# Kudo510/ImageSequenceRegistrationfor6DPoseEstimationLabeling

Hardware: AMD Instinct MI355X
Metric: registered images/sec (T-LESS obj 1-like, synthetic) + final Chamfer error (higher is better)
Workload: dtype bf16

## Files before the change

imagesequenceregistrationfor6dposeestimationlabeling_amd/_capi.py:

```python
from __future__ import annotations

import ctypes as C
from pathlib import Path

import torch

import os

_PKG = Path(__file__).resolve().parent
LIB_PATH = Path(os.environ["ISR_HIP_LIB"]) if os.environ.get("ISR_HIP_LIB") else _PKG / "libisr_hip.so"

ISR_OK = 0
ABI_VERSION = 6
DTYPE_BF16 = 0
DTYPE_F32 = 1
DTYPE_BF16_LOG2 = 2
DTYPE_BF16_LOG2_SCREENED = 3
RANSAC_STAGED = 0
RANSAC_SEQUENTIAL = 1
INLIERS_REFIT = 0
INLIERS_RANSAC = 1
FINAL_REFIT = 0
FINAL_EPNP = 1
TUNE = {"nn_path": 0, "nn_filter": 1, "icp_warm": 2, "nn_plan_rq": 3, "nn_plan_blocks": 4,
# ... 131 lines not shown

RADIUS_SIGNATURES = {
    "isr_radius_workspace_bytes": (_sz, [_i]),
    "isr_radius_count": (_i, [_vp, _i, _d, _i, _vp, _vp, _sz, _vp]),
    "isr_radius_count_host": (_i, [_vp, _i, _d, _i, _vp]),
}

KNN_SIGNATURES = {
    "isr_knn_workspace_bytes": (_sz, [_i, _i, _i]),
    "isr_knn": (_i, [_vp, _i, _vp, _i, _i, _vp, _vp, _vp, _sz, _vp]),
    "isr_knn_host": (_i, [_vp, _i, _vp, _i, _i, _vp, _vp]),
    "isr_local_frames": (_i, [_vp, _i, _vp, _i, _i, _vp, _vp, _vp]),
    "isr_local_frames_host": (_i, [_vp, _i, _vp, _i, _i, _vp, _vp]),
}

_RAYS_SPEC = [_i, _vp, _vp, _vp, _vp, _i, _i, _i, _i, _i, _f, _f, _f, _f, _f, _f, _i, _u64]
RAYS_SIGNATURES = {
    "isr_rays_workspace_bytes": (_sz, [_i, _i]),
    "isr_rays_bundle": (_i, [*_RAYS_SPEC, _vp, _vp, _vp, _vp, _vp]),
    "isr_rays_bundle_host": (_i, [*_RAYS_SPEC, _vp, _vp, _vp, _vp]),
    "isr_rays_select_count": (_i, [*_RAYS_SPEC, _vp, _i, _i, _vp, _vp, _sz, _vp]),
    "isr_rays_select_emit": (_i, [*_RAYS_SPEC, _vp, _i, _i, _vp, _sz, _i64, _vp, _vp, _vp, _vp, _vp, _vp]),
    "isr_rays_select_count_host": (_i, [*_RAYS_SPEC, _vp, _i, _i, _vp]),
    "isr_rays_select_emit_host": (_i, [*_RAYS_SPEC, _vp, _i, _i, _i64, _vp, _vp, _vp, _vp, _vp]),
    "isr_sample_nearest": (_i, [_vp, _i, _i, _i, _i, _vp, _i, _vp, _vp]),
    "isr_sample_nearest_host": (_i, [_vp, _i, _i, _i, _i, _vp, _i, _vp]),
    "isr_rays_philox_host": (_i, [_vp, _vp, _vp, _vp]),
}

_RADIANCE_FIELD = [_vp, _sz, _i, _vp, _i, _i, _i]
# ... 66 lines not shown
    if _lib is not None:
        return _lib
    if not LIB_PATH.exists():
        raise IsrError(
            f"{LIB_PATH} is missing: build it with "
            "`python -m imagesequenceregistrationfor6dposeestimationlabeling_amd.build` "
            "(there is no CPU fallback)")
    try:
        L = C.CDLL(str(LIB_PATH))
    except OSError as e:
        raise IsrError(f"cannot load {LIB_PATH}: {e}") from e
    for name, (res, args) in {**SIGNATURES, **FIELD_SIGNATURES, **FPS_SIGNATURES, **DENSITY_SIGNATURES,
                               **DENSITY_DIR_SIGNATURES, **RADIUS_SIGNATURES, **MC_SIGNATURES, **KNN_SIGNATURES,
                               **RAYS_SIGNATURES, **RADIANCE_SIGNATURES, **RESAMPLE_SIGNATURES,
                               **CONTRASTIVE_SIGNATURES, **FIELD_GRAD_SIGNATURES, **SAMPLE_GRAD_SIGNATURES,
                               **EA_GRAD_SIGNATURES}.items():
        try:
            fn = getattr(L, name)
        except AttributeError as e:
            raise IsrError(f"{LIB_PATH} does not export {name}") from e
        fn.restype = res
        fn.argtypes = args
    if L.isr_abi_version() != ABI_VERSION:
        raise IsrError(f"ABI version {L.isr_abi_version()} != {ABI_VERSION}")
    _lib = L
    return L


def check(rc: int, what: str) -> None:
    if rc != ISR_OK:
        msg = lib().isr_last_error()
# ... 30 lines not shown
```

imagesequenceregistrationfor6dposeestimationlabeling_amd/csrc/nn_batched.hip:

```cpp
#include "isr_common.hpp"

#include <cstddef>
#include <cstdlib>

namespace {

#ifndef ISR_NN_PACKED_BATCH
#define ISR_NN_PACKED_BATCH 1
#endif
constexpr int kThreads = 256;
constexpr int kTile = 256;
constexpr int kGroup = 8;
constexpr int kNV = 18;

__device__ __forceinline__ void xform64(const double* __restrict__ T, float x, float y, float z,
                                        double& ox, double& oy, double& oz) {
  if (T == nullptr) {
    ox = x; oy = y; oz = z;
    return;
  }
  const double dx = x, dy = y, dz = z;
  ox = fma(T[2], dz, fma(T[1], dy, fma(T[0], dx, T[3])));
  oy = fma(T[6], dz, fma(T[5], dy, fma(T[4], dx, T[7])));
  oz = fma(T[10], dz, fma(T[9], dy, fma(T[8], dx, T[11])));
// ... 886 lines not shown
    else
      nn_finalize_kernel<false><<<fgrid, kThreads, 0, stream>>>(qry, Nq, tgt, Tq, Tt, p.nsplit,
                                                                radius, part_d2, part_idx, b0,
                                                                nn_idx, nn_d, part_sums, nullptr, packed);
    ISR_CHECK_LAUNCH("nn_finalize_kernel");
  }
  if (sum_d || sum_d2 || n_in || cov) {
    const dim3 rblock(32, 8);
    nn_reduce_kernel<<<(B + 7) / 8, rblock, 0, stream>>>(part_sums, p.fblocks, B, sum_d, sum_d2,
                                                         n_in, cov);
    ISR_CHECK_LAUNCH("nn_reduce_kernel");
  }
  return ISR_OK;
}

extern "C" int isr_add_metric(const float* verts, int V, const double* Ta, const double* Tb, int B,
                              double* mean_out, isr_stream_t stream) {
  ISR_REQUIRE(verts && mean_out, "isr_add_metric: null pointer");
  ISR_REQUIRE(V > 0 && B > 0, "isr_add_metric: V=%d B=%d", V, B);
  add_metric_kernel<<<B, kThreads, 0, isr::as_stream(stream)>>>(verts, V, Ta, Tb, mean_out);
  ISR_CHECK_LAUNCH("add_metric_kernel");
  return ISR_OK;
}

extern "C" size_t isr_icp_workspace_bytes(int Ns, int Nt) {
  if (Ns <= 0 || Nt <= 0) return 0;
  const NNPlan p = make_plan(Ns, Nt, 1, true);
  return isr::align_up((size_t)p.fblocks * kNV * sizeof(double), 256) + isr::align_up((size_t)Ns * 8, 256) +
         2 * isr::align_up((size_t)Ns * 4, 256) + isr::align_up((size_t)((Nt + kTile - 1) / kTile) * 6 * sizeof(float), 256) + 2048;
}
// ... 93 lines not shown
```

imagesequenceregistrationfor6dposeestimationlabeling_amd/csrc/nn_grid.hpp:

```cpp
#pragma once

constexpr int kMaxCells = 1 << 20;
constexpr int kMaxRing = 8;

struct GridDesc {
  double gmin[3];
  double h, inv_h;
  int nx, ny, nz, ncell;
};

__global__ __launch_bounds__(1024) void grid_bbox_kernel(const float* __restrict__ tgt, int Nt, double cell_scale,
                                                         GridDesc* __restrict__ g, int32_t* __restrict__ unresolved) {
  __shared__ float smin[3][16], smax[3][16];
  float lo[3] = {3.0e38f, 3.0e38f, 3.0e38f}, hi[3] = {-3.0e38f, -3.0e38f, -3.0e38f};
  for (int j = threadIdx.x; j < Nt; j += blockDim.x) {
#pragma unroll
    for (int a = 0; a < 3; ++a) {
      const float v = tgt[3 * (size_t)j + a];
      lo[a] = fminf(lo[a], v);
      hi[a] = fmaxf(hi[a], v);
    }
  }
#pragma unroll
  for (int a = 0; a < 3; ++a) {
#pragma unroll
    for (int o = 32; o >= 1; o >>= 1) {
      lo[a] = fminf(lo[a], __shfl_xor(lo[a], o, 64));
      hi[a] = fmaxf(hi[a], __shfl_xor(hi[a], o, 64));
// ... 18 lines not shown
    if ((double)nx * ny * nz <= (double)kMaxCells) break;
    h *= 1.26;
  }
  g->h = h; g->inv_h = 1.0 / h;
  g->nx = nx; g->ny = ny; g->nz = nz; g->ncell = nx * ny * nz;
  if (unresolved) *unresolved = 0;
}

__device__ __forceinline__ int grid_axis_cell(double v, double gmin, double inv_h, int n) {
  const double c = floor((v - gmin) * inv_h);
  return c < 0.0 ? 0 : (c > (double)(n - 1) ? n - 1 : (int)c);
}

__global__ __launch_bounds__(kThreads) void grid_count_kernel(const float* __restrict__ tgt, int Nt,
                                                              const GridDesc* __restrict__ g,
                                                              int32_t* __restrict__ cid, int32_t* __restrict__ count) {
  const int j = blockIdx.x * kThreads + threadIdx.x;
  if (j >= Nt) return;
  const int cx = grid_axis_cell(tgt[3 * (size_t)j], g->gmin[0], g->inv_h, g->nx);
  const int cy = grid_axis_cell(tgt[3 * (size_t)j + 1], g->gmin[1], g->inv_h, g->ny);
  const int cz = grid_axis_cell(tgt[3 * (size_t)j + 2], g->gmin[2], g->inv_h, g->nz);
  const int c = (cz * g->ny + cy) * g->nx + cx;
  cid[j] = c;
  atomicAdd(&count[c], 1);
}

__global__ __launch_bounds__(1024) void grid_scan_kernel(const GridDesc* __restrict__ g, const int32_t* __restrict__ count,
                                                         int32_t* __restrict__ start) {
  __shared__ int32_t part[1024];
  const int n = g->ncell;
  const int per = (n + 1023) / 1024;
  const int lo = threadIdx.x * per, hi = min(n, lo + per);
  int32_t s = 0;
  for (int i = lo; i < hi; ++i) s += count[i];
  part[threadIdx.x] = s;
  __syncthreads();
  for (int o = 1; o < 1024; o <<= 1) {
    const int32_t v = threadIdx.x >= o ? part[threadIdx.x - o] : 0;
    __syncthreads();
    part[threadIdx.x] += v;
    __syncthreads();
  }
  int32_t run = threadIdx.x ? part[threadIdx.x - 1] : 0;
  for (int i = lo; i < hi; ++i) { start[i] = run; run += count[i]; }
  if (threadIdx.x == 1023) start[n] = part[1023];
}

__global__ __launch_bounds__(kThreads) void grid_scatter_kernel(const float* __restrict__ tgt, int Nt,
                                                                const int32_t* __restrict__ cid,
                                                                const int32_t* __restrict__ start,
                                                                int32_t* __restrict__ count, float4* __restrict__ sorted) {
  const int j = blockIdx.x * kThreads + threadIdx.x;
  if (j >= Nt) return;
  const int c = cid[j];
  const int pos = start[c] + atomicSub(&count[c], 1) - 1;
  sorted[pos] = make_float4(tgt[3 * (size_t)j], tgt[3 * (size_t)j + 1], tgt[3 * (size_t)j + 2], __int_as_float(j));
}

__global__ __launch_bounds__(kThreads) void nn_grid_search_kernel(
    const float* __restrict__ qry, int Nq, const GridDesc* __restrict__ g, const int32_t* __restrict__ start,
    const float4* __restrict__ sorted, const double* __restrict__ Tq, const double* __restrict__ Tt,
    float stop_radius, float* __restrict__ part_d2, int32_t* __restrict__ part_idx,
    int32_t* __restrict__ unresolved, const int32_t* __restrict__ skip) {
  if (skip && *skip) return;
  const int b = blockIdx.y;
  const int qi = blockIdx.x * kThreads + threadIdx.x;
// ... 83 lines not shown
  } else {
    part_idx[o] = kUnresolved;
    atomicAdd(unresolved, 1);
  }
}

constexpr int kTileRings = 10;
constexpr int kTileRuns = 1024;

struct QBlock {
  int32_t start, count;
};

__global__ __launch_bounds__(kThreads) void qblocks_count_kernel(const GridDesc* __restrict__ g,
                                                                 const int32_t* __restrict__ start, int tb,
                                                                 int32_t* __restrict__ nblk) {
  const int c = blockIdx.x * kThreads + threadIdx.x;
  if (c >= g->ncell) return;
  nblk[c] = (start[c + 1] - start[c] + tb - 1) / tb;
}

__global__ __launch_bounds__(kThreads) void qblocks_fill_kernel(const GridDesc* __restrict__ g,
                                                                const int32_t* __restrict__ start,
                                                                const int32_t* __restrict__ bstart, int tb,
                                                                QBlock* __restrict__ table) {
  const int c = blockIdx.x * kThreads + threadIdx.x;
  if (c >= g->ncell) return;
  const int s0 = start[c], cnt = start[c + 1] - s0;
  int o = bstart[c];
  for (int j = 0; j < cnt; j += tb) table[o++] = QBlock{s0 + j, min(tb, cnt - j)};
}

template <int TB>
__device__ __forceinline__ float block_reduce_max(float v, float* red) {
#pragma unroll
  for (int o = 32; o >= 1; o >>= 1) v = fmaxf(v, __shfl_xor(v, o, 64));
  if (TB == 64) return v;
  __syncthreads();
  if ((threadIdx.x & 63) == 0) red[threadIdx.x >> 6] = v;
  __syncthreads();
  float m = red[0];
#pragma unroll
  for (int w = 1; w < TB / 64; ++w) m = fmaxf(m, red[w]);
  return m;
}

template <int TB>
__global__ __launch_bounds__(TB) void nn_tile_search_kernel(
    const float4* __restrict__ qsorted, const QBlock* __restrict__ qtable, const GridDesc* __restrict__ gq,
    const int32_t* __restrict__ qbstart, int Nq, const GridDesc* __restrict__ g, const int32_t* __restrict__ start,
    const float4* __restrict__ sorted, int Nt, const double* __restrict__ Tq, const double* __restrict__ Tt, int nb,
    float stop_radius, float* __restrict__ part_d2, int32_t* __restrict__ part_idx, const int32_t* __restrict__ skip) {
  __shared__ __attribute__((aligned(16))) float tile[3][kTile];
  __shared__ int32_t tidx[kTile];
  __shared__ int32_t run_start[kTileRuns], run_pref[kTileRuns + 1];
  __shared__ float red[TB / 64];
  __shared__ int32_t scan_w[TB / 64];
  if (skip && *skip) return;
  const int tid = threadIdx.x;
  const int nqb = qbstart[gq->ncell];
  const int nx = g->nx, ny = g->ny, nz = g->nz;
  const double gh = g->h, ginv = g->inv_h;
  const float h = (float)gh;

  for (long item = blockIdx.x; item < (long)nqb * nb; item += gridDim.x) {
    const int b = (int)(item / nqb);
    const QBlock qb = qtable[item % nqb];
    const double* tq = Tq ? Tq + 12 * (size_t)b : nullptr;
    const double* tt = Tt ? Tt + 12 * (size_t)b : nullptr;
    const bool valid = tid < qb.count;
    const float4 qp = qsorted[qb.start + (valid ? tid : 0)];
    const int qorig = __float_as_int(qp.w);
    double x, y, z;
    xform64(tq, qp.x, qp.y, qp.z, x, y, z);
    const float qx = (float)x, qy = (float)y, qz = (float)z;

    double mx = qx, my = qy, mz = qz;
    bool rigid = true;
    if (tt) {
      const double r00 = tt[0], r01 = tt[1], r02 = tt[2], r10 = tt[4], r11 = tt[5], r12 = tt[6], r20 = tt[8],
                   r21 = tt[9], r22 = tt[10];
      const double g00 = r00 * r00 + r10 * r10 + r20 * r20, g11 = r01 * r01 + r11 * r11 + r21 * r21,
                   g22 = r02 * r02 + r12 * r12 + r22 * r22, g01 = r00 * r01 + r10 * r11 + r20 * r21,
                   g02 = r00 * r02 + r10 * r12 + r20 * r22, g12 = r01 * r02 + r11 * r12 + r21 * r22;
      const double dev = fmax(fmax(fmax(fabs(g00 - 1.0), fabs(g11 - 1.0)), fabs(g22 - 1.0)),
                              fmax(fmax(fabs(g01), fabs(g02)), fabs(g12)));
      rigid = dev < 3.0e-3;
// ... 209 lines not shown
         isr::align_up((size_t)(Nq + 1) * sizeof(QBlock), 256);
}

GridWs take_grid(isr::Workspace& w, int Nt) {
  GridWs g;
  char* head = w.take<char>(isr::align_up(sizeof(GridDesc) + 64, 256));
  g.desc = reinterpret_cast<GridDesc*>(head);
  g.unresolved = reinterpret_cast<int32_t*>(head + isr::align_up(sizeof(GridDesc), 16));
  g.count = w.take<int32_t>(kMaxCells + 1);
  g.start = w.take<int32_t>(kMaxCells + 1);
  g.cid = w.take<int32_t>(Nt);
  g.sorted = w.take<float4>(Nt);
  return g;
}

void build_grid(const GridWs& g, const float* tgt, int Nt, hipStream_t stream, double cell_scale = 2.5) {
  (void)hipMemsetAsync(g.count, 0, (size_t)(kMaxCells + 1) * 4, stream);
  grid_bbox_kernel<<<1, 1024, 0, stream>>>(tgt, Nt, cell_scale, g.desc, g.unresolved);
  const int nb = (Nt + kThreads - 1) / kThreads;
  grid_count_kernel<<<nb, kThreads, 0, stream>>>(tgt, Nt, g.desc, g.cid, g.count);
  grid_scan_kernel<<<1, 1024, 0, stream>>>(g.desc, g.count, g.start);
  grid_scatter_kernel<<<nb, kThreads, 0, stream>>>(tgt, Nt, g.cid, g.start, g.count, g.sorted);
}

TileWs take_tile(isr::Workspace& w, int Nq, int Nt) {
  TileWs tw;
  tw.t = take_grid(w, Nt);
  tw.q = take_grid(w, Nq);
  tw.bstart = w.take<int32_t>(kMaxCells + 1);
  tw.table = w.take<QBlock>(Nq + 1);
  return tw;
}

struct TileCfg {
  double st, sq;
  int tb;
};

TileCfg tile_cfg() {
  TileCfg c{kCellScaleTgt, kCellScaleQry, kTileTB};
  if (const int v = isr::tuning(ISR_TUNE_NN_TILE_ST); v > 0) c.st = v * 1e-3;
  if (const int v = isr::tuning(ISR_TUNE_NN_TILE_SQ); v > 0) c.sq = v * 1e-3;
  if (const int v = isr::tuning(ISR_TUNE_NN_TILE_TB); v > 0) c.tb = v;
  if (c.tb != 64 && c.tb != 128 && c.tb != 256) c.tb = kTileTB;
  return c;
}

void build_tile(const TileWs& tw, const float* qry, int Nq, const float* tgt, int Nt, hipStream_t stream) {
  const TileCfg cfg = tile_cfg();
  const double st = cfg.st, sq = cfg.sq;
  const int tb = cfg.tb;
  build_grid(tw.t, tgt, Nt, stream, st);
  build_grid(tw.q, qry, Nq, stream, sq);
  const int cb = (kMaxCells + kThreads - 1) / kThreads;
  (void)hipMemsetAsync(tw.q.count, 0, (size_t)(kMaxCells + 1) * 4, stream);
  qblocks_count_kernel<<<cb, kThreads, 0, stream>>>(tw.q.desc, tw.q.start, tb, tw.q.count);
  grid_scan_kernel<<<1, 1024, 0, stream>>>(tw.q.desc, tw.q.count, tw.bstart);
  qblocks_fill_kernel<<<cb, kThreads, 0, stream>>>(tw.q.desc, tw.q.start, tw.bstart, tb, tw.table);
}

void launch_tile_search(const TileWs& tw, int Nq, int Nt, const double* tq, const double* tt, int nb, float stop_radius,
                        float* part_d2, int32_t* part_idx, const int32_t* skip, hipStream_t stream) {
  const int tb = tile_cfg().tb;
#define ISR_TILE_LAUNCH(TBv)                                                                                      \
  nn_tile_search_kernel<TBv><<<kTileGrid * (kThreads / TBv), TBv, 0, stream>>>(                                   \
      tw.q.sorted, tw.table, tw.q.desc, tw.bstart, Nq, tw.t.desc, tw.t.start, tw.t.sorted, Nt, tq, tt, nb,        \
      stop_radius, part_d2, part_idx, skip)
  if (tb == 64) ISR_TILE_LAUNCH(64);
  else if (tb == 128) ISR_TILE_LAUNCH(128);
  else ISR_TILE_LAUNCH(256);
#undef ISR_TILE_LAUNCH
}
```

imagesequenceregistrationfor6dposeestimationlabeling_amd/ops.py:

```python
from __future__ import annotations

import ctypes
from dataclasses import dataclass

import numpy as np

import torch

from . import _capi
from ._capi import check, current_stream, lib, ptr, require_cuda

_workspaces: dict[tuple, torch.Tensor] = {}

_timers: dict[str, list] | None = None


def enable_timing(on: bool = True) -> None:
    global _timers
    _timers = {} if on else None


def drain_timing() -> dict[str, tuple[int, float, float]]:
    out = {}
    if _timers is None:
# ... 15 lines not shown
            self.e0 = torch.cuda.Event(enable_timing=True)
            self.e1 = torch.cuda.Event(enable_timing=True)
            self.e0.record()
        return self

    def __exit__(self, *exc):
        if _timers is not None:
            self.e1.record()
            _timers.setdefault(self.name, []).append((self.e0, self.e1, self.work))
        return False


class tuning:

    def __init__(self, **knobs):
        self.knobs = {_capi.TUNE[k]: int(v) for k, v in knobs.items()}

    def __enter__(self):
        L = lib()
        self.old = {k: L.isr_tuning_get(k) for k in self.knobs}
        for k, v in self.knobs.items():
            check(L.isr_tuning_set(k, v), "isr_tuning_set")
        return self

    def __exit__(self, *exc):
        L = lib()
        for k, v in self.old.items():
            L.isr_tuning_set(k, v)
        return False


def set_tuning(**knobs) -> None:
    for k, v in knobs.items():
        check(lib().isr_tuning_set(_capi.TUNE[k], int(v)), "isr_tuning_set")


def set_tile_plan(plan: str | None) -> None:
    if plan is None:
        set_tuning(nn_tile_st=0, nn_tile_sq=0, nn_tile_tb=0)
    else:
        st, sq, tb = plan.split(",")
        set_tuning(nn_tile_st=round(float(st) * 1000), nn_tile_sq=round(float(sq) * 1000), nn_tile_tb=int(tb))


def workspace(device: torch.device, nbytes: int, tag: str = "default") -> torch.Tensor:
    key = (device.index, torch.cuda.current_stream(device).cuda_stream, tag)
    buf = _workspaces.get(key)
    if buf is not None and buf.numel() >= nbytes:
        return buf
# ... 45 lines not shown
    L = lib()
    sum_d = torch.empty(B, dtype=torch.float64, device=dev)
    sum_d2 = torch.empty(B, dtype=torch.float64, device=dev)
    n_in = torch.empty(B, dtype=torch.int32, device=dev)
    nn_idx = torch.empty((B, Nq), dtype=torch.int32, device=dev) if want_idx else None
    nn_d = torch.empty((B, Nq), dtype=torch.float64, device=dev) if want_dist else None
    cov = torch.empty((B, 16), dtype=torch.float64, device=dev) if want_cov else None
    nbytes = L.isr_nn_batched_workspace_bytes(Nq, Nt, B)
    ws = workspace(dev, nbytes, "nn")
    with torch.cuda.device(dev), _timed("nn_batched", float(B) * Nq * Nt):
        rc = L.isr_nn_batched(ptr(qry), Nq, ptr(tgt), Nt, ptr(Tq), ptr(Tt), B, float(radius),
                              ptr(sum_d), ptr(sum_d2), ptr(n_in), ptr(nn_idx), ptr(nn_d), ptr(cov),
                              ptr(ws), ws.numel(), current_stream(dev))
    check(rc, "isr_nn_batched")
    return NNResult(sum_d, sum_d2, n_in, nn_idx, nn_d, cov)


def icp_point_to_point_batch(sources: torch.Tensor, target: torch.Tensor, state: torch.Tensor, threshold: float,
                             max_iter: int = 30, rel_fitness: float = 1e-6, rel_rmse: float = 1e-6) -> torch.Tensor:
    dev = require_cuda(sources, target, state)
    if sources.dtype != torch.float32 or target.dtype != torch.float32 or not (sources.is_contiguous() and target.is_contiguous()):
        raise ValueError("icp_point_to_point_batch: sources and target must be contiguous float32")
    if state.dtype != torch.float64 or state.ndim != 2 or state.shape[1] != 20 or not state.is_contiguous():
        raise ValueError(f"icp_point_to_point_batch: state must be contiguous (B,20) float64, got {tuple(state.shape)} {state.dtype}")
    if target.ndim != 2 or target.shape[1] != 3 or sources.ndim not in (2, 3) or sources.shape[-1] != 3:
        raise ValueError(f"icp_point_to_point_batch: sources {tuple(sources.shape)} must be (Ns,3) or (B,Ns,3), target "
                         f"{tuple(target.shape)} (Nt,3)")
    B, Ns, Nt = state.shape[0], sources.shape[-2], target.shape[0]
    if sources.ndim == 3 and sources.shape[0] != B:
        raise ValueError(f"icp_point_to_point_batch: sources {tuple(sources.shape)} and state {tuple(state.shape)} disagree on B")
# ... 1804 lines not shown
```

imagesequenceregistrationfor6dposeestimationlabeling_amd/registration.py:

```python
from __future__ import annotations

import numpy as np
import torch

from . import ops
from ._capi import IsrError

SOLVEPNP_P3P = 2
SOLVEPNP_AP3P = 5

_state = {"surface_pts": None, "device": None}


def device() -> torch.device:
    if not torch.cuda.is_available():
        raise IsrError("no HIP device visible: the registration hot path has no CPU fallback")
    return torch.device("cuda", torch.cuda.current_device())


def _dev(x, dtype=None) -> torch.Tensor:
    if isinstance(x, torch.Tensor):
        t = x if x.is_cuda else x.to(device())
    else:
        t = torch.from_numpy(np.ascontiguousarray(x)).to(device())
# ... 138 lines not shown
    ab = ops.nn_batched(a, b, ta, tb)
    ba = ops.nn_batched(b, a, tb, ta)
    return 0.5 * (float(ab.sum_d.item()) / a.shape[0] + float(ba.sum_d.item()) / b.shape[0])


def chamfer_pairs(pc1, R_pred, R_rel_gt):
    pc = _dev(pc1, torch.float32)
    Rp = np.asarray(R_pred, np.float64)
    Rr = np.asarray(R_rel_gt, np.float64)
    n1 = Rp.shape[0] - 1
    Tg = np.zeros((n1, 3, 4))
    Tp = np.zeros((n1, 3, 4))
    Tg[:, :, :3] = np.einsum("nji,njk->nik", Rr, Rp[:-1])
    Tp[:, :, :3] = np.transpose(Rp[1:], (0, 2, 1))
    tg, tp = _dev(Tg.reshape(n1, 12)), _dev(Tp.reshape(n1, 12))
    ab = ops.nn_batched(pc, pc, tp, tg)
    ba = ops.nn_batched(pc, pc, tg, tp)
    return 0.5 * (ab.sum_d + ba.sum_d) / pc.shape[0]


def choose_best(chamferdis):
    c = chamferdis.cpu().numpy() if isinstance(chamferdis, torch.Tensor) else np.asarray(chamferdis)
    i = int(np.argmin(c))
    return i, float(c[i])


def _eval(src, tgt, threshold, T):
    dev = src.device
    Tq = torch.from_numpy(np.ascontiguousarray(np.asarray(T, np.float64)[:3, :].reshape(1, 12))).to(dev)
    buf = torch.empty(18, dtype=torch.float64, device=dev)
    Nq, Nt = src.shape[0], tgt.shape[0]
    L = ops.lib()
    ws = ops.workspace(dev, L.isr_nn_batched_workspace_bytes(Nq, Nt, 1), "nn")
# ... 167 lines not shown
```

Baseline: 1095.

## Add neighbour-table self-NN path for chamfer between pose-transformed copies of one cloud

Adds a self-nearest-neighbour routine for chamfer between two rigidly transformed copies of the same cloud. It uses a cached per-cloud KNN table and squared radius to resolve most queries cheaply, and runs the exact grid/tile search only for unresolved queries through a device-side 'need' flag. The grid build and tile search kernels gain early-exit guards that read this flag. A Python gate routes to the new path only when most relative rotations are small. This adds KNN table construction, a cache keyed per cloud, and extra kernel launches, and correctness depends on the fallback resolving all misses.

```diff
diff --git a/imagesequenceregistrationfor6dposeestimationlabeling_amd/_capi.py b/imagesequenceregistrationfor6dposeestimationlabeling_amd/_capi.py
--- a/imagesequenceregistrationfor6dposeestimationlabeling_amd/_capi.py
+++ b/imagesequenceregistrationfor6dposeestimationlabeling_amd/_capi.py
@@ -169,6 +169,13 @@
     "isr_local_frames_host": (_i, [_vp, _i, _vp, _i, _i, _vp, _vp]),
 }
 
+NN_SELF_SIGNATURES = {
+    "isr_nn_self_batched_workspace_bytes": (_sz, [_i, _i, _i]),
+    "isr_nn_self_batched": (_i, [_vp, _i, _vp, _vp, _i, _vp, _vp, _i, _d, _vp, _vp, _vp, _vp, _vp, _vp, _vp, _sz, _vp]),
+    "isr_nn_self_search_host": (_i, [_vp, _i, _vp, _vp, _i, _vp, _vp, _i, _vp, _vp, _vp]),
+    "isr_nn_self_unresolved": (_i, [_vp, _sz, _i, _vp, _vp, _vp]),
+}
+
 _RAYS_SPEC = [_i, _vp, _vp, _vp, _vp, _i, _i, _i, _i, _i, _f, _f, _f, _f, _f, _f, _i, _u64]
 RAYS_SIGNATURES = {
     "isr_rays_workspace_bytes": (_sz, [_i, _i]),
@@ -265,7 +272,7 @@
                                **DENSITY_DIR_SIGNATURES, **RADIUS_SIGNATURES, **MC_SIGNATURES, **KNN_SIGNATURES,
                                **RAYS_SIGNATURES, **RADIANCE_SIGNATURES, **RESAMPLE_SIGNATURES,
                                **CONTRASTIVE_SIGNATURES, **FIELD_GRAD_SIGNATURES, **SAMPLE_GRAD_SIGNATURES,
-                               **EA_GRAD_SIGNATURES}.items():
+                               **EA_GRAD_SIGNATURES, **NN_SELF_SIGNATURES}.items():
         try:
             fn = getattr(L, name)
         except AttributeError as e:
diff --git a/imagesequenceregistrationfor6dposeestimationlabeling_amd/csrc/nn_batched.hip b/imagesequenceregistrationfor6dposeestimationlabeling_amd/csrc/nn_batched.hip
--- a/imagesequenceregistrationfor6dposeestimationlabeling_amd/csrc/nn_batched.hip
+++ b/imagesequenceregistrationfor6dposeestimationlabeling_amd/csrc/nn_batched.hip
@@ -1,4 +1,6 @@
 #include "isr_common.hpp"
+#include "nn_self.hpp"
+#include "../../include/isr_nn_self.h"
 
 #include <cstddef>
 #include <cstdlib>
@@ -924,6 +926,83 @@
   return ISR_OK;
 }
 
+namespace {
+NNPlan make_self_plan(int N, int B) {
+  NNPlan p = make_plan(N, N, B);
+  if (p.grid) p.grid = false;
+  p.nsplit = 1;
+  p.split_len = ((N + kTile - 1) / kTile) * kTile;
+  long bc = (long)(kPartBudget / ((size_t)N * 8));
+  p.bchunk = (int)(bc < 1 ? 1 : (bc > B ? B : (bc > 65535 ? 65535 : bc)));
+  return p;
+}
+}
+
+extern "C" size_t isr_nn_self_batched_workspace_bytes(int N, int K, int B) {
+  if (N <= 0 || B <= 0 || K < 1 || K > isr::nn_self::kMaxK || K > N) return 0;
+  const NNPlan p = make_self_plan(N, B);
+  size_t n = isr::nn_self::head_bytes(B);
+  n += isr::align_up((size_t)p.bchunk * N * sizeof(float), 256);
+  n += isr::align_up((size_t)p.bchunk * N * sizeof(int32_t), 256);
+  n += isr::align_up((size_t)B * p.fblocks * kNV * sizeof(double), 256);
+  n += tile_ws_bytes(N, N);
+  return n + 256;
+}
+
+extern "C" int isr_nn_self_batched(const float* pts, int N, const int32_t* nbr, const float* r2, int K, const double* Tq,
+                                   const double* Tt, int B, double radius, double* sum_d, double* sum_d2, int32_t* n_in,
+                                   int32_t* nn_idx, double* nn_d, double* cov, void* ws, size_t ws_bytes, isr_stream_t stream_) {
+  ISR_REQUIRE(pts && nbr && r2, "isr_nn_self_batched: null cloud or table pointer");
+  ISR_REQUIRE(N > 0 && B > 0, "isr_nn_self_batched: N=%d B=%d must be positive", N, B);
+  ISR_REQUIRE(K >= 1 && K <= isr::nn_self::kMaxK && K <= N, "isr_nn_self_batched: K=%d (1..min(N = %d, %d))", K, N,
+              isr::nn_self::kMaxK);
+  ISR_REQUIRE(sum_d || sum_d2 || n_in || nn_idx || nn_d || cov, "isr_nn_self_batched: no output requested");
+  if (!ws || ws_bytes < isr_nn_self_batched_workspace_bytes(N, K, B)) {
+    isr::set_error("isr_nn_self_batched: workspace %zu < %zu", ws_bytes, isr_nn_self_batched_workspace_bytes(N, K, B));
+    return ISR_ERR_WORKSPACE;
+  }
+  hipStream_t stream = isr::as_stream(stream_);
+  const NNPlan p = make_self_plan(N, B);
+  isr::Workspace w(ws, ws_bytes);
+  const isr::nn_self::Head head = isr::nn_self::take_head(w, B);
+  float* part_d2 = w.take<float>((size_t)p.bchunk * N);
+  int32_t* part_idx = w.take<int32_t>((size_t)p.bchunk * N);
+  double* part_sums = w.take<double>((size_t)B * p.fblocks * kNV);
+  TileWs tw{};
+  if (p.tile) tw = take_tile(w, N, N);
+  const float stop_radius = (radius >= 0.0 && !nn_d) ? (float)(radius * (1.0 + 1e-6)) : -1.f;
+
+  for (int b0 = 0; b0 < B; b0 += p.bchunk) {
+    const int nb = (B - b0 < p.bchunk) ? (B - b0) : p.bchunk;
+    const double* tq = Tq ? Tq + 12 * (size_t)b0 : nullptr;
+    const double* tt = Tt ? Tt + 12 * (size_t)b0 : nullptr;
+    if (int rc = isr::nn_self::enqueue(pts, N, nbr, r2, K, Tq, Tt, B, b0, nb, head, part_d2, part_idx, stream)) return rc;
+    if (p.tile) {
+      build_tile(tw, pts, N, pts, N, stream, head.counts);
+      ISR_CHECK_LAUNCH("tile grid build");
+      launch_tile_search(tw, N, N, tq, tt, nb, stop_radius, part_d2, part_idx, nullptr, stream, head.counts, b0);
+    } else {
+      launch_search(p, dim3(p.qblocks, 1, nb), stream, pts, N, pts, N, tq, tt, part_d2, part_idx, nullptr, head.counts, nullptr,
+                    nullptr);
+    }
+    ISR_CHECK_LAUNCH("nn_self exact search");
+    const dim3 fgrid(p.fblocks, nb);
+    if (cov)
+      nn_finalize_kernel<true><<<fgrid, kThreads, 0, stream>>>(pts, N, pts, Tq, Tt, 1, radius, part_d2, part_idx, b0, nn_idx, nn_d,
+                                                               part_sums, nullptr, nullptr);
+    else
+      nn_finalize_kernel<false><<<fgrid, kThreads, 0, stream>>>(pts, N, pts, Tq, Tt, 1, radius, part_d2, part_idx, b0, nn_idx, nn_d,
+                                                                part_sums, nullptr, nullptr);
+    ISR_CHECK_LAUNCH("nn_finalize_kernel");
+  }
+  if (sum_d || sum_d2 || n_in || cov) {
+    const dim3 rblock(32, 8);
+    nn_reduce_kernel<<<(B + 7) / 8, rblock, 0, stream>>>(part_sums, p.fblocks, B, sum_d, sum_d2, n_in, cov);
+    ISR_CHECK_LAUNCH("nn_reduce_kernel");
+  }
+  return ISR_OK;
+}
+
 extern "C" int isr_add_metric(const float* verts, int V, const double* Ta, const double* Tb, int B,
                               double* mean_out, isr_stream_t stream) {
   ISR_REQUIRE(verts && mean_out, "isr_add_metric: null pointer");
diff --git a/imagesequenceregistrationfor6dposeestimationlabeling_amd/csrc/nn_grid.hpp b/imagesequenceregistrationfor6dposeestimationlabeling_amd/csrc/nn_grid.hpp
--- a/imagesequenceregistrationfor6dposeestimationlabeling_amd/csrc/nn_grid.hpp
+++ b/imagesequenceregistrationfor6dposeestimationlabeling_amd/csrc/nn_grid.hpp
@@ -10,8 +10,10 @@
 };
 
 __global__ __launch_bounds__(1024) void grid_bbox_kernel(const float* __restrict__ tgt, int Nt, double cell_scale,
-                                                         GridDesc* __restrict__ g, int32_t* __restrict__ unresolved) {
+                                                         GridDesc* __restrict__ g, int32_t* __restrict__ unresolved,
+                                                         const int32_t* __restrict__ need = nullptr) {
   __shared__ float smin[3][16], smax[3][16];
+  if (need && *need == 0) return;
   float lo[3] = {3.0e38f, 3.0e38f, 3.0e38f}, hi[3] = {-3.0e38f, -3.0e38f, -3.0e38f};
   for (int j = threadIdx.x; j < Nt; j += blockDim.x) {
 #pragma unroll
@@ -60,7 +62,9 @@
 
 __global__ __launch_bounds__(kThreads) void grid_count_kernel(const float* __restrict__ tgt, int Nt,
                                                               const GridDesc* __restrict__ g,
-                                                              int32_t* __restrict__ cid, int32_t* __restrict__ count) {
+                                                              int32_t* __restrict__ cid, int32_t* __restrict__ count,
+                                                              const int32_t* __restrict__ need = nullptr) {
+  if (need && *need == 0) return;
   const int j = blockIdx.x * kThreads + threadIdx.x;
   if (j >= Nt) return;
   const int cx = grid_axis_cell(tgt[3 * (size_t)j], g->gmin[0], g->inv_h, g->nx);
@@ -72,8 +76,10 @@
 }
 
 __global__ __launch_bounds__(1024) void grid_scan_kernel(const GridDesc* __restrict__ g, const int32_t* __restrict__ count,
-                                                         int32_t* __restrict__ start) {
+                                                         int32_t* __restrict__ start,
+                                                         const int32_t* __restrict__ need = nullptr) {
   __shared__ int32_t part[1024];
+  if (need && *need == 0) return;
   const int n = g->ncell;
   const int per = (n + 1023) / 1024;
   const int lo = threadIdx.x * per, hi = min(n, lo + per);
@@ -95,7 +101,9 @@
 __global__ __launch_bounds__(kThreads) void grid_scatter_kernel(const float* __restrict__ tgt, int Nt,
                                                                 const int32_t* __restrict__ cid,
                                                                 const int32_t* __restrict__ start,
-                                                                int32_t* __restrict__ count, float4* __restrict__ sorted) {
+                                                                int32_t* __restrict__ count, float4* __restrict__ sorted,
+                                                                const int32_t* __restrict__ need = nullptr) {
+  if (need && *need == 0) return;
   const int j = blockIdx.x * kThreads + threadIdx.x;
   if (j >= Nt) return;
   const int c = cid[j];
@@ -209,7 +217,9 @@
 
 __global__ __launch_bounds__(kThreads) void qblocks_count_kernel(const GridDesc* __restrict__ g,
                                                                  const int32_t* __restrict__ start, int tb,
-                                                                 int32_t* __restrict__ nblk) {
+                                                                 int32_t* __restrict__ nblk,
+                                                                 const int32_t* __restrict__ need = nullptr) {
+  if (need && *need == 0) return;
   const int c = blockIdx.x * kThreads + threadIdx.x;
   if (c >= g->ncell) return;
   nblk[c] = (start[c + 1] - start[c] + tb - 1) / tb;
@@ -218,7 +228,9 @@
 __global__ __launch_bounds__(kThreads) void qblocks_fill_kernel(const GridDesc* __restrict__ g,
                                                                 const int32_t* __restrict__ start,
                                                                 const int32_t* __restrict__ bstart, int tb,
-                                                                QBlock* __restrict__ table) {
+                                                                QBlock* __restrict__ table,
+                                                                const int32_t* __restrict__ need = nullptr) {
+  if (need && *need == 0) return;
   const int c = blockIdx.x * kThreads + threadIdx.x;
   if (c >= g->ncell) return;
   const int s0 = start[c], cnt = start[c + 1] - s0;
@@ -240,18 +252,20 @@
   return m;
 }
 
-template <int TB>
+template <int TB, bool NEED = false>
 __global__ __launch_bounds__(TB) void nn_tile_search_kernel(
     const float4* __restrict__ qsorted, const QBlock* __restrict__ qtable, const GridDesc* __restrict__ gq,
     const int32_t* __restrict__ qbstart, int Nq, const GridDesc* __restrict__ g, const int32_t* __restrict__ start,
     const float4* __restrict__ sorted, int Nt, const double* __restrict__ Tq, const double* __restrict__ Tt, int nb,
-    float stop_radius, float* __restrict__ part_d2, int32_t* __restrict__ part_idx, const int32_t* __restrict__ skip) {
+    float stop_radius, float* __restrict__ part_d2, int32_t* __restrict__ part_idx, const int32_t* __restrict__ skip,
+    const int32_t* __restrict__ need = nullptr, int need_b0 = 0) {
   __shared__ __attribute__((aligned(16))) float tile[3][kTile];
   __shared__ int32_t tidx[kTile];
   __shared__ int32_t run_start[kTileRuns], run_pref[kTileRuns + 1];
   __shared__ float red[TB / 64];
   __shared__ int32_t scan_w[TB / 64];
   if (skip && *skip) return;
+  if (NEED && need[0] == 0) return;
   const int tid = threadIdx.x;
   const int nqb = qbstart[gq->ncell];
   const int nx = g->nx, ny = g->ny, nz = g->nz;
@@ -260,12 +274,14 @@
 
   for (long item = blockIdx.x; item < (long)nqb * nb; item += gridDim.x) {
     const int b = (int)(item / nqb);
+    if (NEED && need[1 + need_b0 + b] == 0) continue;
     const QBlock qb = qtable[item % nqb];
     const double* tq = Tq ? Tq + 12 * (size_t)b : nullptr;
     const double* tt = Tt ? Tt + 12 * (size_t)b : nullptr;
     const bool valid = tid < qb.count;
     const float4 qp = qsorted[qb.start + (valid ? tid : 0)];
     const int qorig = __float_as_int(qp.w);
+    if (NEED && !__syncthreads_or(valid && part_idx[(size_t)b * Nq + qorig] == kUnresolved)) continue;
     double x, y, z;
     xform64(tq, qp.x, qp.y, qp.z, x, y, z);
     const float qx = (float)x, qy = (float)y, qz = (float)z;
@@ -505,13 +521,14 @@
   return g;
 }
 
-void build_grid(const GridWs& g, const float* tgt, int Nt, hipStream_t stream, double cell_scale = 2.5) {
+void build_grid(const GridWs& g, const float* tgt, int Nt, hipStream_t stream, double cell_scale = 2.5,
+                const int32_t* need = nullptr) {
   (void)hipMemsetAsync(g.count, 0, (size_t)(kMaxCells + 1) * 4, stream);
-  grid_bbox_kernel<<<1, 1024, 0, stream>>>(tgt, Nt, cell_scale, g.desc, g.unresolved);
+  grid_bbox_kernel<<<1, 1024, 0, stream>>>(tgt, Nt, cell_scale, g.desc, g.unresolved, need);
   const int nb = (Nt + kThreads - 1) / kThreads;
-  grid_count_kernel<<<nb, kThreads, 0, stream>>>(tgt, Nt, g.desc, g.cid, g.count);
-  grid_scan_kernel<<<1, 1024, 0, stream>>>(g.desc, g.count, g.start);
-  grid_scatter_kernel<<<nb, kThreads, 0, stream>>>(tgt, Nt, g.cid, g.start, g.count, g.sorted);
+  grid_count_kernel<<<nb, kThreads, 0, stream>>>(tgt, Nt, g.desc, g.cid, g.count, need);
+  grid_scan_kernel<<<1, 1024, 0, stream>>>(g.desc, g.count, g.start, need);
+  grid_scatter_kernel<<<nb, kThreads, 0, stream>>>(tgt, Nt, g.cid, g.start, g.count, g.sorted, need);
 }
 
 TileWs take_tile(isr::Workspace& w, int Nq, int Nt) {
@@ -537,28 +554,36 @@
   return c;
 }
 
-void build_tile(const TileWs& tw, const float* qry, int Nq, const float* tgt, int Nt, hipStream_t stream) {
+void build_tile(const TileWs& tw, const float* qry, int Nq, const float* tgt, int Nt, hipStream_t stream,
+                const int32_t* need = nullptr) {
   const TileCfg cfg = tile_cfg();
   const double st = cfg.st, sq = cfg.sq;
   const int tb = cfg.tb;
-  build_grid(tw.t, tgt, Nt, stream, st);
-  build_grid(tw.q, qry, Nq, stream, sq);
+  build_grid(tw.t, tgt, Nt, stream, st, need);
+  build_grid(tw.q, qry, Nq, stream, sq, need);
   const int cb = (kMaxCells + kThreads - 1) / kThreads;
   (void)hipMemsetAsync(tw.q.count, 0, (size_t)(kMaxCells + 1) * 4, stream);
-  qblocks_count_kernel<<<cb, kThreads, 0, stream>>>(tw.q.desc, tw.q.start, tb, tw.q.count);
-  grid_scan_kernel<<<1, 1024, 0, stream>>>(tw.q.desc, tw.q.count, tw.bstart);
-  qblocks_fill_kernel<<<cb, kThreads, 0, stream>>>(tw.q.desc, tw.q.start, tw.bstart, tb, tw.table);
+  qblocks_count_kernel<<<cb, kThreads, 0, stream>>>(tw.q.desc, tw.q.start, tb, tw.q.count, need);
+  grid_scan_kernel<<<1, 1024, 0, stream>>>(tw.q.desc, tw.q.count, tw.bstart, need);
+  qblocks_fill_kernel<<<cb, kThreads, 0, stream>>>(tw.q.desc, tw.q.start, tw.bstart, tb, tw.table, need);
 }
 
 void launch_tile_search(const TileWs& tw, int Nq, int Nt, const double* tq, const double* tt, int nb, float stop_radius,
-                        float* part_d2, int32_t* part_idx, const int32_t* skip, hipStream_t stream) {
+                        float* part_d2, int32_t* part_idx, const int32_t* skip, hipStream_t stream,
+                        const int32_t* need = nullptr, int need_b0 = 0) {
   const int tb = tile_cfg().tb;
-#define ISR_TILE_LAUNCH(TBv)                                                                                      \
-  nn_tile_search_kernel<TBv><<<kTileGrid * (kThreads / TBv), TBv, 0, stream>>>(                                   \
+#define ISR_TILE_LAUNCH(TBv, NEEDv)                                                                               \
+  nn_tile_search_kernel<TBv, NEEDv><<<kTileGrid * (kThreads / TBv), TBv, 0, stream>>>(                            \
       tw.q.sorted, tw.table, tw.q.desc, tw.bstart, Nq, tw.t.desc, tw.t.start, tw.t.sorted, Nt, tq, tt, nb,        \
-      stop_radius, part_d2, part_idx, skip)
-  if (tb == 64) ISR_TILE_LAUNCH(64);
-  else if (tb == 128) ISR_TILE_LAUNCH(128);
-  else ISR_TILE_LAUNCH(256);
+      stop_radius, part_d2, part_idx, skip, need, need_b0)
+  if (need) {
+    if (tb == 64) ISR_TILE_LAUNCH(64, true);
+    else if (tb == 128) ISR_TILE_LAUNCH(128, true);
+    else ISR_TILE_LAUNCH(256, true);
+    return;
+  }
+  if (tb == 64) ISR_TILE_LAUNCH(64, false);
+  else if (tb == 128) ISR_TILE_LAUNCH(128, false);
+  else ISR_TILE_LAUNCH(256, false);
 #undef ISR_TILE_LAUNCH
 }
diff --git a/imagesequenceregistrationfor6dposeestimationlabeling_amd/csrc/nn_self.hip b/imagesequenceregistrationfor6dposeestimationlabeling_amd/csrc/nn_self.hip
--- /dev/null
+++ b/imagesequenceregistrationfor6dposeestimationlabeling_amd/csrc/nn_self.hip
@@ -0,0 +1,93 @@
+#include "nn_self.hpp"
+
+#include "../../include/isr_nn_self.h"
+
+namespace {
+
+using namespace isr::nn_self;
+
+constexpr int kThreads = 256;
+
+__global__ __launch_bounds__(kThreads) void nn_self_items_kernel(const double* __restrict__ Tt, int B, Item* __restrict__ items,
+                                                                 int32_t* __restrict__ counts) {
+  const int b = blockIdx.x * kThreads + threadIdx.x;
+  if (b <= B) counts[b] = 0;
+  if (b < B) items[b] = item_bounds(Tt ? Tt + 12 * (size_t)b : nullptr);
+}
+
+__global__ __launch_bounds__(kThreads) void nn_self_search_kernel(const float* __restrict__ pts, int N, const int32_t* __restrict__ nbr,
+                                                                  const float* __restrict__ r2, int K, const double* __restrict__ Tq,
+                                                                  const double* __restrict__ Tt, int b0, const Item* __restrict__ items,
+                                                                  float* __restrict__ part_d2, int32_t* __restrict__ part_idx,
+                                                                  int32_t* __restrict__ counts) {
+  const int bl = blockIdx.y, b = b0 + bl;
+  const int j = blockIdx.x * kThreads + threadIdx.x;
+  bool unres = false;
+  if (j < N) {
+    float best;
+    int bidx;
+    const bool ok = search(pts, N, nbr + (size_t)j * K, r2[j], K, j, Tq ? Tq + 12 * (size_t)b : nullptr,
+                           Tt ? Tt + 12 * (size_t)b : nullptr, items[b], best, bidx);
+    const size_t o = (size_t)bl * N + j;
+    part_d2[o] = best;
+    part_idx[o] = ok ? bidx : kUnresolved;
+    unres = !ok;
+  }
+  const unsigned long long m = __ballot(unres);
+  if (m != 0 && (threadIdx.x & 63) == 0) {
+    const int n = __popcll(m);
+    atomicAdd(&counts[0], n);
+    atomicAdd(&counts[1 + b], n);
+  }
+}
+
+}
+
+int isr::nn_self::enqueue(const float* pts, int N, const int32_t* nbr, const float* r2, int K, const double* Tq, const double* Tt,
+                          int B, int b0, int nb, const Head& head, float* part_d2, int32_t* part_idx, hipStream_t stream) {
+  if (b0 == 0) {
+    nn_self_items_kernel<<<(B + 1 + kThreads - 1) / kThreads, kThreads, 0, stream>>>(Tt, B, head.items, head.counts);
+    ISR_CHECK_LAUNCH("nn_self_items_kernel");
+  }
+  nn_self_search_kernel<<<dim3((N + kThreads - 1) / kThreads, nb), kThreads, 0, stream>>>(pts, N, nbr, r2, K, Tq, Tt, b0, head.items,
+                                                                                         part_d2, part_idx, head.counts);
+  ISR_CHECK_LAUNCH("nn_self_search_kernel");
+  return ISR_OK;
+}
+
+extern "C" int isr_nn_self_search_host(const float* pts, int N, const int32_t* nbr, const float* r2, int K, const double* Tq,
+                                       const double* Tt, int B, float* part_d2, int32_t* part_idx, int32_t* unresolved) {
+  ISR_REQUIRE(pts && nbr && r2 && part_d2 && part_idx && unresolved, "isr_nn_self_search_host: null pointer");
+  ISR_REQUIRE(N > 0 && B > 0 && K >= 1 && K <= kMaxK && K <= N, "isr_nn_self_search_host: N=%d B=%d K=%d (K in 1..min(N, %d))", N, B, K,
+              kMaxK);
+  for (int b = 0; b < B; ++b) {
+    const double* tq = Tq ? Tq + 12 * (size_t)b : nullptr;
+    const double* tt = Tt ? Tt + 12 * (size_t)b : nullptr;
+    const Item it = item_bounds(tt);
+    isr::parallel_rows(N, 512, [=](long j) {
+      float best;
+      int bidx;
+      const bool ok = search(pts, N, nbr + (size_t)j * K, r2[j], K, (int)j, tq, tt, it, best, bidx);
+      part_d2[(size_t)b * N + j] = best;
+      part_idx[(size_t)b * N + j] = ok ? bidx : kUnresolved;
+    });
+    int n = 0;
+    for (int j = 0; j < N; ++j) n += part_idx[(size_t)b * N + j] == kUnresolved;
+    unresolved[b] = n;
+  }
+  return ISR_OK;
+}
+
+extern "C" int isr_nn_self_unresolved(const void* ws, size_t ws_bytes, int B, int32_t* total_host, int32_t* per_item_host,
+                                      isr_stream_t stream_) {
+  ISR_REQUIRE(ws && total_host && B > 0, "isr_nn_self_unresolved: null pointer or B=%d", B);
+  ISR_REQUIRE(ws_bytes >= head_bytes(B), "isr_nn_self_unresolved: workspace %zu < %zu", ws_bytes, head_bytes(B));
+  isr::Workspace w(const_cast<void*>(ws), ws_bytes);
+  const Head head = take_head(w, B);
+  hipStream_t stream = isr::as_stream(stream_);
+  ISR_CHECK_HIP(hipMemcpyAsync(total_host, head.counts, sizeof(int32_t), hipMemcpyDeviceToHost, stream));
+  if (per_item_host)
+    ISR_CHECK_HIP(hipMemcpyAsync(per_item_host, head.counts + 1, (size_t)B * sizeof(int32_t), hipMemcpyDeviceToHost, stream));
+  ISR_CHECK_HIP(hipStreamSynchronize(stream));
+  return ISR_OK;
+}
diff --git a/imagesequenceregistrationfor6dposeestimationlabeling_amd/csrc/nn_self.hpp b/imagesequenceregistrationfor6dposeestimationlabeling_amd/csrc/nn_self.hpp
--- /dev/null
+++ b/imagesequenceregistrationfor6dposeestimationlabeling_amd/csrc/nn_self.hpp
@@ -0,0 +1,127 @@
+#pragma once
+#include <cmath>
+#include <cstddef>
+#include <cstdint>
+
+#if defined(__HIPCC__)
+#include "isr_common.hpp"
+#define ISR_NNS_FN __host__ __device__ inline
+#else
+#define ISR_NNS_FN inline
+#endif
+
+namespace isr {
+namespace nn_self {
+
+constexpr int kUnresolved = -2;
+constexpr int kMaxK = 64;
+constexpr double kEtaMax = 0.009;
+constexpr float kTiny = 1e-18f;
+
+struct Item {
+  float inv1m;
+  float tau;
+};
+
+ISR_NNS_FN void xform(const double* T, const float* p, double& ox, double& oy, double& oz) {
+  const double dx = p[0], dy = p[1], dz = p[2];
+  if (T == nullptr) {
+    ox = dx; oy = dy; oz = dz;
+    return;
+  }
+  ox = fma(T[2], dz, fma(T[1], dy, fma(T[0], dx, T[3])));
+  oy = fma(T[6], dz, fma(T[5], dy, fma(T[4], dx, T[7])));
+  oz = fma(T[10], dz, fma(T[9], dy, fma(T[8], dx, T[11])));
+}
+
+ISR_NNS_FN float d32(float qx, float qy, float qz, float tx, float ty, float tz) {
+  const float dx = qx - tx, dy = qy - ty, dz = qz - tz;
+  return fmaf(dz, dz, fmaf(dy, dy, dx * dx));
+}
+
+ISR_NNS_FN Item item_bounds(const double* tt) {
+  Item it;
+  it.inv1m = 1.f;
+  it.tau = 0.f;
+  if (tt == nullptr) return it;
+  double g = 0.0;
+  for (int a = 0; a < 3; ++a)
+    for (int b = a; b < 3; ++b) {
+      const double s = tt[a] * tt[b] + tt[4 + a] * tt[4 + b] + tt[8 + a] * tt[8 + b] - (a == b ? 1.0 : 0.0);
+      g = fmax(g, fabs(s));
+      if (s != s) g = s;
+    }
+  const double eta = 3.0 * g + 1e-9;
+  const double tau = sqrt(tt[3] * tt[3] + tt[7] * tt[7] + tt[11] * tt[11]);
+  const bool ok = (eta <= kEtaMax) && (tau < 1e30);
+  it.inv1m = ok ? (float)(1.0 / (1.0 - eta)) * 1.000001f : 0.f;
+  it.tau = ok ? (float)tau * 1.000001f : 0.f;
+  return it;
+}
+
+ISR_NNS_FN int clamp_index(int c, int N) { return c < 0 ? 0 : (c < N ? c : N - 1); }
+
+ISR_NNS_FN bool search(const float* pts, int N, const int32_t* row, float r2j, int K, int j, const double* tq,
+                       const double* tt, Item it, float& best, int& bidx) {
+  double x, y, z;
+  xform(tq, pts + 3 * (size_t)j, x, y, z);
+  const float qx = (float)x, qy = (float)y, qz = (float)z;
+  xform(tt, pts + 3 * (size_t)j, x, y, z);
+  const float jx = (float)x, jy = (float)y, jz = (float)z;
+  const float Dj = d32(qx, qy, qz, jx, jy, jz);
+  best = Dj;
+  bidx = j;
+  auto candidate = [&](int c) {
+    c = clamp_index(c, N);
+    double cx, cy, cz;
+    xform(tt, pts + 3 * (size_t)c, cx, cy, cz);
+    const float d = d32(qx, qy, qz, (float)cx, (float)cy, (float)cz);
+    const bool up = (d < best) | ((d == best) & (c < bidx));
+    best = up ? d : best;
+    bidx = up ? c : bidx;
+  };
+  int k = 0;
+#if defined(__HIP_DEVICE_COMPILE__)
+  if ((((uintptr_t)row) & 15) == 0)
+    for (; k + 4 <= K; k += 4) {
+      const int4 v = *reinterpret_cast<const int4*>(row + k);
+      candidate(v.x);
+      candidate(v.y);
+      candidate(v.z);
+      candidate(v.w);
+    }
+#endif
+  for (; k < K; ++k) candidate(row[k]);
+
+  const float S = (sqrtf(best) + sqrtf(Dj)) * 1.000001f + kTiny;
+  const float tn = sqrtf(fmaf(jz, jz, fmaf(jy, jy, jx * jx)));
+  const float E = (1.01f * 5.9604645e-8f) * (2.f * tn + S + 2.f * it.tau);
+  const float P = (S + E) * it.inv1m * 1.00001f;
+  return (it.inv1m > 0.f) & (r2j > 0.f) & (P * P * 1.00001f < r2j);
+}
+
+}
+}
+
+#if defined(__HIPCC__)
+namespace isr {
+namespace nn_self {
+
+struct Head {
+  int32_t* counts;
+  Item* items;
+};
+inline Head take_head(Workspace& w, int B) {
+  Head h;
+  h.counts = w.take<int32_t>((size_t)B + 1);
+  h.items = w.take<Item>((size_t)B);
+  return h;
+}
+inline size_t head_bytes(int B) { return align_up(((size_t)B + 1) * 4, 256) + align_up((size_t)B * sizeof(Item), 256); }
+
+int enqueue(const float* pts, int N, const int32_t* nbr, const float* r2, int K, const double* Tq, const double* Tt, int B, int b0,
+            int nb, const Head& head, float* part_d2, int32_t* part_idx, hipStream_t stream);
+
+}
+}
+#endif
diff --git a/imagesequenceregistrationfor6dposeestimationlabeling_amd/ops.py b/imagesequenceregistrationfor6dposeestimationlabeling_amd/ops.py
--- a/imagesequenceregistrationfor6dposeestimationlabeling_amd/ops.py
+++ b/imagesequenceregistrationfor6dposeestimationlabeling_amd/ops.py
@@ -53,6 +53,7 @@
 class tuning:
 
     def __init__(self, **knobs):
+        self.py_knobs = {k: int(knobs.pop(k)) for k in list(knobs) if k in py_knobs}
         self.knobs = {_capi.TUNE[k]: int(v) for k, v in knobs.items()}
 
     def __enter__(self):
@@ -60,18 +61,27 @@
         self.old = {k: L.isr_tuning_get(k) for k in self.knobs}
         for k, v in self.knobs.items():
             check(L.isr_tuning_set(k, v), "isr_tuning_set")
+        self.py_old = {k: py_knobs[k] for k in self.py_knobs}
+        py_knobs.update(self.py_knobs)
         return self
 
     def __exit__(self, *exc):
         L = lib()
         for k, v in self.old.items():
             L.isr_tuning_set(k, v)
+        py_knobs.update(self.py_old)
         return False
+
+
+py_knobs: dict[str, int] = {"nn_self": 1}
 
 
 def set_tuning(**knobs) -> None:
     for k, v in knobs.items():
-        check(lib().isr_tuning_set(_capi.TUNE[k], int(v)), "isr_tuning_set")
+        if k in py_knobs:
+            py_knobs[k] = int(v)
+        else:
+            check(lib().isr_tuning_set(_capi.TUNE[k], int(v)), "isr_tuning_set")
 
 
 def set_tile_plan(plan: str | None) -> None:
@@ -147,6 +157,85 @@
                               ptr(ws), ws.numel(), current_stream(dev))
     check(rc, "isr_nn_batched")
     return NNResult(sum_d, sum_d2, n_in, nn_idx, nn_d, cov)
+
+
+_last_nn_self = None
+
+
+def nn_batched_self(pts: torch.Tensor, nbr: torch.Tensor, r2: torch.Tensor, Tq: torch.Tensor | None = None,
+                    Tt: torch.Tensor | None = None, radius: float = -1.0, want_idx: bool = False,
+                    want_dist: bool = False, want_cov: bool = False) -> NNResult:
+    global _last_nn_self
+    dev = require_cuda(pts, nbr, r2, Tq, Tt)
+    pts, Tq, Tt = _f32c(pts), _f64c(Tq), _f64c(Tt)
+    if pts.ndim != 2 or pts.shape[1] != 3:
+        raise ValueError(f"cloud must be (N,3): got {tuple(pts.shape)}")
+    N = pts.shape[0]
+    if nbr.dtype != torch.int32 or nbr.ndim != 2 or nbr.shape[0] != N or not nbr.is_contiguous():
+        raise ValueError(f"nbr must be contiguous (N,K) int32 with N = {N}, got {tuple(nbr.shape)} {nbr.dtype}")
+    if r2.dtype != torch.float32 or r2.shape != (N,) or not r2.is_contiguous():
+        raise ValueError(f"r2 must be contiguous (N,) float32 with N = {N}, got {tuple(r2.shape)} {r2.dtype}")
+    K = nbr.shape[1]
+    B = 1
+    for T in (Tq, Tt):
+        if T is not None:
+            if T.numel() % 12:
+                raise ValueError("transforms must be (B,3,4)")
+            B = max(B, T.numel() // 12)
+    for T in (Tq, Tt):
+        if T is not None and T.numel() // 12 != B:
+            raise ValueError("Tq and Tt must have the same batch size")
+    L = lib()
+    sum_d = torch.empty(B, dtype=torch.float64, device=dev)
+    sum_d2 = torch.empty(B, dtype=torch.float64, device=dev)
+    n_in = torch.empty(B, dtype=torch.int32, device=dev)
+    nn_idx = torch.empty((B, N), dtype=torch.int32, device=dev) if want_idx else None
+    nn_d = torch.empty((B, N), dtype=torch.float64, device=dev) if want_dist else None
+    cov = torch.empty((B, 16), dtype=torch.float64, device=dev) if want_cov else None
+    nbytes = L.isr_nn_self_batched_workspace_bytes(N, K, B)
+    if nbytes == 0:
+        raise ValueError(f"nn_batched_self: N = {N}, K = {K}, B = {B} refused (K in 1..min(N, 64))")
+    ws = workspace(dev, nbytes, "nn_self")
+    with torch.cuda.device(dev), _timed("nn_batched", float(B) * N * N):
+        rc = L.isr_nn_self_batched(ptr(pts), N, ptr(nbr), ptr(r2), K, ptr(Tq), ptr(Tt), B, float(radius),
+                                   ptr(sum_d), ptr(sum_d2), ptr(n_in), ptr(nn_idx), ptr(nn_d), ptr(cov),
+                                   ptr(ws), ws.numel(), current_stream(dev))
+    check(rc, "isr_nn_self_batched")
+    _last_nn_self = (ws, B, dev)
+    return NNResult(sum_d, sum_d2, n_in, nn_idx, nn_d, cov)
+
+
+def nn_self_unresolved() -> tuple[int, np.ndarray]:
+    if _last_nn_self is None:
+        return -1, np.zeros(0, np.int32)
+    ws, B, dev = _last_nn_self
+    total = ctypes.c_int32(-1)
+    per = np.full(B, -1, np.int32)
+    with torch.cuda.device(dev):
+        rc = lib().isr_nn_self_unresolved(ptr(ws), ws.numel(), B, ctypes.addressof(total), per.ctypes.data, current_stream(dev))
+    check(rc, "isr_nn_self_unresolved")
+    return int(total.value), per
+
+
+def nn_self_search_host(pts, nbr, r2, Tq=None, Tt=None):
+    pts = np.ascontiguousarray(pts, np.float32)
+    nbr = np.ascontiguousarray(nbr, np.int32)
+    r2 = np.ascontiguousarray(r2, np.float32)
+    N, K = nbr.shape
+    B = 1
+    Ts = []
+    for T in (Tq, Tt):
+        T = None if T is None else np.ascontiguousarray(T, np.float64).reshape(-1, 12)
+        if T is not None:
+            B = T.shape[0]
+        Ts.append(T)
+    hp = lambda a: None if a is None else a.ctypes.data_as(ctypes.c_void_p)
+    part_d2 = np.empty((B, N), np.float32)
+    part_idx = np.empty((B, N), np.int32)
+    unres = np.empty(B, np.int32)
+    check(lib().isr_nn_self_search_host(hp(pts), N, hp(nbr), hp(r2), K, hp(Ts[0]), hp(Ts[1]), B, hp(part_d2), hp(part_idx),
+                                        hp(unres)), "isr_nn_self_search_host")
+    return part_idx, part_d2, unres
 
 
 def icp_point_to_point_batch(sources: torch.Tensor, target: torch.Tensor, state: torch.Tensor, threshold: float,
diff --git a/imagesequenceregistrationfor6dposeestimationlabeling_amd/registration.py b/imagesequenceregistrationfor6dposeestimationlabeling_amd/registration.py
--- a/imagesequenceregistrationfor6dposeestimationlabeling_amd/registration.py
+++ b/imagesequenceregistrationfor6dposeestimationlabeling_amd/registration.py
@@ -176,9 +176,44 @@
     Tg[:, :, :3] = np.einsum("nji,njk->nik", Rr, Rp[:-1])
     Tp[:, :, :3] = np.transpose(Rp[1:], (0, 2, 1))
     tg, tp = _dev(Tg.reshape(n1, 12)), _dev(Tp.reshape(n1, 12))
-    ab = ops.nn_batched(pc, pc, tp, tg)
-    ba = ops.nn_batched(pc, pc, tg, tp)
+    if _table_route(Tg, Tp, pc.shape[0]):
+        nbr, r2 = cloud_neighbours(pc, SELF_K)
+        ab = ops.nn_batched_self(pc, nbr, r2, tp, tg)
+        ba = ops.nn_batched_self(pc, nbr, r2, tg, tp)
+    else:
+        ab = ops.nn_batched(pc, pc, tp, tg)
+        ba = ops.nn_batched(pc, pc, tg, tp)
     return 0.5 * (ab.sum_d + ba.sum_d) / pc.shape[0]
+
+
+SELF_MIN_POINTS = 1024
+SELF_K = 16
+SELF_GATE = 0.35
+_nbr_cache: dict = {}
+
+
+def _table_route(Tg, Tp, N) -> bool:
+    mode = ops.py_knobs["nn_self"]
+    if N < SELF_MIN_POINTS or mode == 0:
+        return False
+    if mode == 2:
+        return True
+    rel = np.einsum("nji,njk->nik", Tg[:, :, :3], Tp[:, :, :3])
+    ang = np.arccos(np.clip(0.5 * (np.trace(rel, axis1=1, axis2=2) - 1.0), -1.0, 1.0))
+    return 2 * int(np.count_nonzero(ang <= SELF_GATE * np.sqrt(SELF_K / N))) >= len(ang)
+
+
+def cloud_neighbours(pc: torch.Tensor, K: int = SELF_K):
+    from .sequence import cloud_key
+    pc = pc.to(torch.float32).contiguous()
+    key = cloud_key(pc) + (int(K),)
+    tab = _nbr_cache.get(key)
+    if tab is None:
+        if len(_nbr_cache) > 4:
+            _nbr_cache.clear()
+        nbr, d2 = ops.knn(pc, pc, int(K), check_finite=False)
+        tab = _nbr_cache[key] = (nbr, d2[:, -1].contiguous())
+    return tab
 
 
 def choose_best(chamferdis):
diff --git a/include/isr_nn_self.h b/include/isr_nn_self.h
--- /dev/null
+++ b/include/isr_nn_self.h
@@ -0,0 +1,29 @@
+#ifndef ISR_NN_SELF_H
+#define ISR_NN_SELF_H
+
+#include <stddef.h>
+#include <stdint.h>
+
+#include "isr_hip.h"
+
+#ifdef __cplusplus
+extern "C" {
+#endif
+
+size_t isr_nn_self_batched_workspace_bytes(int N, int K, int B);
+
+int isr_nn_self_batched(const float* pts, int N, const int32_t* nbr, const float* r2, int K, const double* Tq, const double* Tt,
+                        int B, double radius, double* sum_d, double* sum_d2, int32_t* n_in, int32_t* nn_idx, double* nn_d,
+                        double* cov, void* ws, size_t ws_bytes, isr_stream_t stream);
+
+int isr_nn_self_search_host(const float* pts, int N, const int32_t* nbr, const float* r2, int K, const double* Tq,
+                            const double* Tt, int B, float* part_d2, int32_t* part_idx, int32_t* unresolved);
+
+int isr_nn_self_unresolved(const void* ws, size_t ws_bytes, int B, int32_t* total_host, int32_t* per_item_host,
+                           isr_stream_t stream);
+
+#ifdef __cplusplus
+}
+#endif
+
+#endif
```

Result: no change. 1095 (-0.0%).
